# microsoft/demikernel

Hardware: AMD Instinct MI355X
Metric: GB/s packet bytes checksummed+parsed (device-resident) (higher is better)
Workload: dtype u8; 1 GPU; 1M x 1500B IPv4/TCP, 1024 flows, device-resident; frames_per_gpu=1048576, global_frames=1048576, parallelism=packet-shard x1, collective=none

## Files before the change

### demikernel_amd/csrc/tcp_kernels.hip

```cpp
#include <hip/hip_runtime.h>
#include <rocprim/device/device_radix_sort.hpp>
#include <rocprim/iterator/counting_iterator.hpp>
#include <rocprim/warp/warp_scan.hpp>

#include <algorithm>
#include <climits>
#include <cerrno>
#include <cstdlib>
#include <cstddef>
#include <cstring>

#include "../../include/dk_diag.h"
#include "../../include/dk_tcp.h"
#include "tcp_order.h"

namespace dk_tcp {
namespace {

constexpr uint32_t kBlock = 256;
constexpr uint32_t kBatch = 8;

using SortConfig = rocprim::radix_sort_config<rocprim::default_config, rocprim::default_config,
                                              rocprim::default_config, 0>;

__device__ __forceinline__ bool lt(uint32_t a, uint32_t b) { return (int32_t)(a - b) < 0; }
__device__ __forceinline__ bool le(uint32_t a, uint32_t b) { return (int32_t)(a - b) <= 0; }
__device__ __forceinline__ bool ge(uint32_t a, uint32_t b) { return (int32_t)(a - b) >= 0; }

struct Params {
    const uint32_t* meta;
    const uint32_t* flow_id;
    const uint32_t* seq;
    const uint32_t* ack;
    const uint32_t* payload;
    uint32_t n;
    dk_tcp_conn* conns;
    uint32_t nconns;
    uint32_t* keys;
    uint32_t* skeys;
    uint32_t* svals;
    uint4* rec;
    uint32_t* range;
    uint32_t* cls;
    uint32_t* open_until;
    uint4* scan_sum;
    int* scan_ends;
    uint32_t* scan_idx;
    uint4* scan_rec;
    uint4* scan_post;
    uint32_t* scan_head;
    uint32_t* shape;
    uint32_t* shape_host;
    uint32_t call;
    dk_tcp_out out;
};
constexpr uint32_t kNoConn = 0xFFFFFFFFu;

__global__ __launch_bounds__(kBlock) void dk_tcp_key_kernel(Params P) {
    const uint32_t i = blockIdx.x * kBlock + threadIdx.x;
    if (i >= P.n) return;
    const uint32_t meta = P.meta[i], pay = P.payload[i], seq = P.seq[i];
    uint32_t key = 2 * P.nconns, cls = kNoConn;
    uint8_t act = DK_TCP_SKIP;
    if ((meta & 0xFFu) == DK_V_OK_TCP) {
        const uint32_t f = P.flow_id[i];
        if (f < P.nconns) {
            static_assert(offsetof(dk_tcp_conn, state) == 0 && offsetof(dk_tcp_conn, receive_next) == 4 &&
                              offsetof(dk_tcp_conn, reader_next) == 8 && offsetof(dk_tcp_conn, buffer_size) == 12,
                          "dk_tcp_conn layout");
            const uint4 h = *reinterpret_cast<const uint4*>(P.conns + f);
            const uint32_t state = h.x;
            if (state != DK_TCP_NONE) key = 2 * f;
            const uint32_t bufsz = h.w, rn0 = h.y, wend = h.z + bufsz;
            if (state == DK_TCP_ESTABLISHED && wend - rn0 <= bufsz && bufsz < 0x40000000u) {
                const uint32_t flags = (meta >> 16) & 0xFFu, len = pay >> 16;
                const uint32_t full = len + ((flags >> 1) & 1u) + (flags & 1u);
                const uint32_t seg_end = full ? seq + (full - 1) : seq;
                const uint32_t lim = 0x7FFFFFFFu - bufsz - 0x20000u;
                if (seq - wend - 1u < lim) act = DK_TCP_OUT_OF_WINDOW;
                else if (rn0 - seg_end - 1u < lim) act = DK_TCP_DUPLICATE;
                if (act != DK_TCP_SKIP) {
                    cls = f;
                    key = 2 * f + 1;
                }
            }
        }
    }
    P.keys[i] = key;
    P.cls[i] = cls;
    P.rec[i] = make_uint4(seq, P.ack[i], meta, pay);
    if (key == 2 * P.nconns || cls != kNoConn) {
        P.out.action[i] = act;
        P.out.view[i] = dk_tcp_view{i, pay & 0xFFFFu, pay >> 16};
    }
}

constexpr uint32_t kShapeBlocks = 64;
__global__ __launch_bounds__(kBlock) void dk_tcp_fix_kernel(Params P) {
    __shared__ uint32_t s_cnt[kBlock / 64];
    const uint32_t i = blockIdx.x * kBlock + threadIdx.x;
    bool stored = false;
    if (i < P.n) {
        const uint32_t c = P.cls[i];
        if (c != kNoConn && i >= P.open_until[c]) P.out.action[i] = DK_TCP_UNPROCESSED;
        else stored = blockIdx.x < kShapeBlocks && c == kNoConn && P.out.action[i] == DK_TCP_STORED;
    }
    if (blockIdx.x >= kShapeBlocks) return;
    const uint64_t m = __ballot(stored);
    if ((threadIdx.x & 63u) == 0) s_cnt[threadIdx.x / 64] = (uint32_t)__popcll(m);
    __syncthreads();
    if (threadIdx.x == 0) {
        uint32_t sum = 0;
        for (uint32_t w = 0; w < kBlock / 64; w++) sum += s_cnt[w];
        const uint32_t nb = min(gridDim.x, kShapeBlocks);
        const unsigned long long old = atomicAdd(reinterpret_cast<unsigned long long*>(P.shape),
                                                 (1ull << 40) | (unsigned long long)sum);
        if ((uint32_t)(old >> 40) == nb - 1) {
            const uint32_t total = (uint32_t)(old & ((1ull << 40) - 1)) + sum;
            atomicExch(reinterpret_cast<unsigned long long*>(P.shape), 0ull);
            __hip_atomic_store(P.shape_host + 0, total, __ATOMIC_RELAXED, __HIP_MEMORY_SCOPE_SYSTEM);
            __hip_atomic_store(P.shape_host + 1, min(P.n, nb * kBlock), __ATOMIC_RELAXED, __HIP_MEMORY_SCOPE_SYSTEM);
            __hip_atomic_store(P.shape_host + 2, P.call, __ATOMIC_RELAXED, __HIP_MEMORY_SCOPE_SYSTEM);
        }
    }
}

__global__ __launch_bounds__(kBlock) void dk_tcp_range_kernel(Params P) {
    const uint32_t c = blockIdx.x * kBlock + threadIdx.x;
    if (c > 2 * P.nconns) return;
    uint32_t lo = 0, hi = P.n;
    while (lo < hi) {
        const uint32_t mid = lo + (hi - lo) / 2;
        if (P.skeys[mid] < c)
            lo = mid + 1;
        else
            hi = mid;
    }
    P.range[c] = lo;
}

constexpr uint32_t kSortBlock = 512, kSortWaves = kSortBlock / 64, kSortTile = 8192, kSortSub = kSortTile / kSortWaves;
#ifndef DK_TCP_SORT_ROWS
#define DK_TCP_SORT_ROWS 255
#endif
constexpr uint32_t kSortMaxRows = DK_TCP_SORT_ROWS, kSortMaxBuckets = 2 * kSortMaxRows + 1;
struct SortPass {
    const uint32_t* kin;
    const uint32_t* vin;
    uint32_t* kout;
    uint32_t* vout;
    uint32_t* H;
    uint32_t shift, mask, nbuck;
};

__device__ __forceinline__ uint64_t digit_group(uint32_t d, bool live, uint32_t nbits) {
    uint64_t same = __ballot(live);
    for (uint32_t bit = 0; bit < nbits; bit++) {
        const uint64_t ones = __ballot(live && ((d >> bit) & 1u));
        same &= ((d >> bit) & 1u) ? ones : ~ones;
    }
    return same;
}
constexpr uint32_t kSortRounds = kSortSub / 64;
constexpr uint32_t kSortGroupBits = 4;

__device__ __forceinline__ void sort_load_keys(const SortPass& S, uint32_t s0, uint32_t s1, uint32_t lane,
                                               uint32_t (&kr)[kSortRounds]) {
#pragma unroll
    for (uint32_t r = 0; r < kSortRounds; r++) {
        const uint32_t i = s0 + r * 64 + lane;
        kr[r] = i < s1 ? S.kin[i] : 0u;
    }
}
__device__ __forceinline__ void sort_count_keys(const SortPass& S, uint32_t s0, uint32_t s1, uint32_t lane,
                                                const uint32_t (&kr)[kSortRounds], uint32_t* cnt, uint32_t nbits) {
    const uint64_t lt = (1ull << lane) - 1;
#pragma unroll
    for (uint32_t r = 0; r < kSortRounds; r++) {
        const bool live = s0 + r * 64 + lane < s1;
        const uint32_t d = (kr[r] >> S.shift) & S.mask;
        if (nbits <= kSortGroupBits) {
            const uint64_t same = digit_group(d, live, nbits);
            if (live && !(same & lt)) atomicAdd(&cnt[d], (uint32_t)__popcll(same));
        } else if (live) {
            atomicAdd(&cnt[d], 1u);
        }
    }
}

__global__ __launch_bounds__(kSortBlock) void dk_tcp_sort_count_kernel(uint32_t n, SortPass S) {
    __shared__ uint32_t hist[kSortMaxBuckets];
    const uint32_t b = blockIdx.x, nb = gridDim.x, tid = threadIdx.x, lane = tid & 63, wv = tid >> 6;
    const uint32_t nbits = 32u - (uint32_t)__builtin_clz(S.mask | 1u);
    uint32_t kr[kSortRounds];
    const uint32_t s0 = b * kSortTile + wv * kSortSub, s1 = min(n, s0 + kSortSub);
    sort_load_keys(S, s0, s1, lane, kr);
    for (uint32_t k = tid; k < S.nbuck; k += kSortBlock) hist[k] = 0;
    __syncthreads();
    sort_count_keys(S, s0, s1, lane, kr, hist, nbits);
    __syncthreads();
    for (uint32_t k = tid; k < S.nbuck; k += kSortBlock) S.H[(size_t)k * nb + b] = hist[k];
}

constexpr uint32_t kSortScanBlock = 1024, kSortScanPer = 12, kSortScanRow = kSortScanPer + 1;
__global__ __launch_bounds__(kSortScanBlock) void dk_tcp_sort_scan_kernel(uint32_t* H, uint32_t m, uint32_t nb,
                                                                          uint32_t* range) {
// ... 276 lines not shown
    if (data.len > 0 || fin) {
        if (seg_start != w.rn) {
            action = DK_TCP_STORED;
            if (seg_len > 0) {
                if (fin) {
                    seg_len -= 1;
                    w.fin_pending = 1;
                    w.fin_seq = seg_end;
                    seg_end -= 1;
                    fin = false;
                }
                if (seg_len > 0) action = ooo_store(s, w, seg_start, seg_end, data);
            }
        } else {
            action = DK_TCP_DELIVERED;
            if (receive_data(s, w, data, o)) fin = true;
        }
    }
    if (fin) {
        o.push(dk_tcp_view{DK_TCP_REF_EOF, 0, 0}, w);
        w.rn += 1;
        w.state = DK_TCP_CLOSED;
        return DK_TCP_FIN;
    }
    return action;
}

__global__ __launch_bounds__(kWalkBlock) void dk_tcp_walk_kernel(Params P) {
    __shared__ uint32_t lds[4 * DK_TCP_OOO_MAX * kWalkBlock];
    const uint32_t c = blockIdx.x * kWalkBlock + threadIdx.x;
    if (c >= P.nconns) return;
    dk_tcp_conn* t = P.conns + c;
    const uint32_t k0 = P.range[2 * c], cnt = P.range[2 * c + 1] - k0, all = P.range[2 * c + 2] - k0;
    const uint32_t d0 = k0 + DK_TCP_DELIV_EXTRA * c;
    P.out.deliv_start[c] = d0;
    Walk w{t->state, t->receive_next, t->reader_next, t->buffer_size, t->send_next, t->fin_pending, t->fin_seq,
           min(t->ooo_count, DK_TCP_OOO_MAX)};
    Store s{lds + threadIdx.x};
    for (uint32_t k = 0; k < w.nooo; k++) s.set(k, t->ooo_start[k], t->ooo[k]);
    uint32_t open_until = w.state == DK_TCP_ESTABLISHED ? 0xFFFFFFFFu : 0u;
    Out o{P.out.deliv + d0, 0, all + DK_TCP_DELIV_EXTRA};
    uint32_t ia[kBatch], ib[kBatch], ic[kBatch];
    uint4 gb[kBatch], gc[kBatch];
#pragma unroll
    for (uint32_t j = 0; j < kBatch; j++) {
        ib[j] = j < cnt ? P.svals[k0 + j] : 0u;
        ia[j] = kBatch + j < cnt ? P.svals[k0 + kBatch + j] : 0u;
    }
#pragma unroll
    for (uint32_t j = 0; j < kBatch; j++)
        if (j < cnt) gb[j] = P.rec[ib[j]];
    for (uint32_t k = 0; k < cnt; k += kBatch) {
#pragma unroll
        for (uint32_t j = 0; j < kBatch; j++) {
            gc[j] = gb[j];
            ic[j] = ib[j];
        }
        if (k + kBatch < cnt) {
#pragma unroll
            for (uint32_t j = 0; j < kBatch; j++) {
                if (k + kBatch + j < cnt) gb[j] = P.rec[ia[j]];
                ib[j] = ia[j];
            }
        }
        if (k + 2 * kBatch < cnt) {
#pragma unroll
            for (uint32_t j = 0; j < kBatch; j++)
                if (k + 2 * kBatch + j < cnt) ia[j] = P.svals[k0 + k + 2 * kBatch + j];
        }
#pragma unroll
        for (uint32_t j = 0; j < kBatch; j++) {
            if (k + j >= cnt) break;
            if (w.state != DK_TCP_ESTABLISHED) {
                P.out.action[ic[j]] = DK_TCP_UNPROCESSED;
                P.out.view[ic[j]] = dk_tcp_view{ic[j], gc[j].w & 0xFFFFu, gc[j].w >> 16};
                continue;
            }
            dk_tcp_view v;
            P.out.action[ic[j]] = (uint8_t)process(s, w, gc[j], ic[j], o, v);
            P.out.view[ic[j]] = v;
            if (w.state != DK_TCP_ESTABLISHED) open_until = ic[j] + 1;
        }
    }
    P.open_until[c] = open_until;
    t->state = w.state;
    t->receive_next = w.rn;
    t->fin_pending = w.fin_pending;
    t->fin_seq = w.fin_seq;
    t->ooo_count = w.nooo;
    for (uint32_t k = 0; k < DK_TCP_OOO_MAX; k++) {
        const bool live = k < w.nooo;
        t->ooo_start[k] = live ? s.start(k) : 0u;
        t->ooo[k] = live ? s.view(k) : dk_tcp_view{0, 0, 0};
    }
    P.out.deliv_count[c] = o.n;
}

constexpr uint32_t kWave = 64;

using WaveScan = rocprim::warp_scan<uint32_t, kWave>;

constexpr uint32_t kRingH = 6, kIdxSlots = 16, kRecSlots = 8;
static_assert(2 * kRingH + 1 <= kIdxSlots && kRingH + 1 <= kRecSlots, "ring slots cover the windows in flight");
static_assert(2 * kRingH - 2 == 10, "the s_waitcnt immediate below");
typedef __attribute__((address_space(3))) void lds_void;
typedef unsigned u32x4 __attribute__((ext_vector_type(4)));
template <class T>
__device__ __forceinline__ uint32_t lds_addr(T* p) {
    return (uint32_t)(uintptr_t)(__attribute__((address_space(3))) T*)p;
}
__device__ __forceinline__ uint32_t lds_read_u32(uint32_t a) {
    uint32_t v;
    asm volatile("ds_read_b32 %0, %1\n\ts_waitcnt lgkmcnt(0)" : "=v"(v) : "v"(a) : "memory");
    return v;
}
__device__ __forceinline__ void lds_read_window(uint32_t a_i, uint32_t a_g, uint32_t a_f, uint32_t& i, uint4& g,
                                                uint32_t& f) {
    u32x4 q;
    asm volatile("ds_read_b32 %0, %3\n\tds_read_b128 %1, %4\n\tds_read_b32 %2, %5\n\ts_waitcnt lgkmcnt(0)"
                 : "=&v"(i), "=&v"(q), "=&v"(f)
                 : "v"(a_i), "v"(a_g), "v"(a_f)
                 : "memory");
    g = make_uint4(q.x, q.y, q.z, q.w);
}

struct Seg {
    uint32_t x, off, len, dend, seg_end;
    bool have, simple, syn, ack_ok;
    uint8_t fast_action;
    __device__ __forceinline__ Seg(uint4 g, bool have_, uint32_t snd) {
        const uint32_t flags = (g.z >> 16) & 0xFFu;
        x = g.x;
        off = g.w & 0xFFFFu;
        len = g.w >> 16;
        have = have_;
        simple = have && !(flags & 0x07u);
        syn = have && (flags & 0x07u) == 0x02u;
        ack_ok = (flags & 0x10u) && le(g.y, snd);
        fast_action = !(flags & 0x10u) ? DK_TCP_NO_ACK : !ack_ok ? DK_TCP_ACK_UNSENT : len > 0 ? DK_TCP_DELIVERED : DK_TCP_NO_DATA;
        dend = x + len;
        const uint32_t full = len + ((flags >> 1) & 1u) + (flags & 1u);
        seg_end = full ? x + (full - 1) : x;
    }
    __device__ __forceinline__ bool cand(bool beyond, uint32_t wend) const {
        return simple && !beyond && ack_ok && len > 0 && !ge(dend - 1u, wend);
    }
};
struct Verdict {
    bool ok;
    uint8_t act;
    uint32_t voff, vlen;
};
__device__ __forceinline__ Verdict classify(const Seg& q, uint32_t rn, uint32_t wend, bool beyond, uint32_t nooo,
                                            uint32_t front, uint32_t fin_pending, uint32_t fin_seq,
                                            bool syn_reach = false) {
    const bool drains = q.ack_ok && q.len > 0 && ((nooo && q.dend == front) || (fin_pending && q.dend == fin_seq));
    const bool at = q.x == rn, before = lt(q.x, rn), dup = before && lt(q.seg_end, rn);
    const bool oow = !at && !before && ge(q.x, wend);
    const bool past = !at && !before && !oow;
    const bool data_in = !ge(q.dend - 1u, wend), plain = q.simple && !beyond && !drains;
    const bool syn_ok = q.syn && (at || past) && !ge(q.seg_end, wend);
    const uint32_t send1 = q.seg_end + 1u;
    const bool syn_part_ok = syn_reach && q.syn && before && !dup && !ge(q.seg_end, wend) &&
                             !(q.ack_ok && ((nooo && send1 == front) || (fin_pending && send1 == fin_seq)));
    const bool ok = dup || oow || syn_ok || syn_part_ok || (at && plain && (q.len == 0 || data_in)) ||
                    (before && plain && data_in) || (past && beyond) ||
                    (past && q.simple && q.fast_action != DK_TCP_DELIVERED);
// ... 66 lines not shown
            const uint32_t a_f = process(s, w, gf, i_f, o, v);
            if (lane == 0) {
                P.out.action[i_f] = (uint8_t)a_f;
                P.out.view[i_f] = v;
            }
            if (w.state != DK_TCP_ESTABLISHED) open_until = i_f + 1;
            lo = f + 1;
        }
    }
};

__device__ __forceinline__ void ring_walk(const Params& P, WaveWalk& W, uint32_t (&sidx)[kIdxSlots][kWave],
                                          uint4 (&srec)[kRecSlots][kWave], uint32_t k0, uint32_t cnt, uint32_t v0,
                                          uint32_t v1) {
    const uint32_t lane = W.lane, last = cnt ? cnt - 1 : 0u;
    const auto idx_dma = [&](uint32_t u) {
        __builtin_amdgcn_global_load_lds((const void*)(P.svals + k0 + min(u * kWave + lane, last)),
                                         (lds_void*)&sidx[u % kIdxSlots][0], 4, 0, 0);
    };
    const auto rec_dma = [&](uint32_t u, uint32_t fi) {
        __builtin_amdgcn_global_load_lds((const void*)(P.rec + fi), (lds_void*)&srec[u % kRecSlots][0], 16, 0, 0);
    };
    const auto idx_at = [&](uint32_t u) { return lds_addr(&sidx[u % kIdxSlots][lane]); };
    if (v0 >= v1) return;
    for (uint32_t u = v0; u < v0 + kRingH; u++) idx_dma(u);
    asm volatile("s_waitcnt vmcnt(0)" ::: "memory");
    for (uint32_t u = v0; u < v0 + kRingH; u++) {
        rec_dma(u, lds_read_u32(idx_at(u)));
        idx_dma(u + kRingH);
    }
    for (uint32_t v = v0; v < v1; v++) {
        asm volatile("s_waitcnt vmcnt(10)" ::: "memory");
        uint32_t i, fi;
        uint4 g;
        lds_read_window(idx_at(v), lds_addr(&srec[v % kRecSlots][lane]), idx_at(v + kRingH), i, g, fi);
        rec_dma(v + kRingH, fi);
        idx_dma(v + 2 * kRingH);
        W.window(v * kWave, i, g);
    }
    asm volatile("s_waitcnt vmcnt(0)" ::: "memory");
}

#define DK_U(x) (uint32_t) __builtin_amdgcn_readfirstlane((int)(x))

template <bool kRing>
__global__ __launch_bounds__(kWave) void dk_tcp_wave_walk_kernel(Params P) {
    __shared__ WaveScan::storage_type scan_tmp;
    __shared__ uint32_t sidx[kRing ? kIdxSlots : 1][kWave];
    __shared__ uint4 srec[kRing ? kRecSlots : 1][kWave];
    const uint32_t c = blockIdx.x, lane = threadIdx.x;
    dk_tcp_conn* t = P.conns + c;
    const uint32_t k0 = P.range[2 * c], cnt = P.range[2 * c + 1] - k0, all = P.range[2 * c + 2] - k0;
    const uint32_t d0 = k0 + DK_TCP_DELIV_EXTRA * c;
    const Walk w0{DK_U(t->state), DK_U(t->receive_next), DK_U(t->reader_next), DK_U(t->buffer_size),
                  DK_U(t->send_next), DK_U(t->fin_pending), DK_U(t->fin_seq), DK_U(min(t->ooo_count, DK_TCP_OOO_MAX))};
    RegStore s0{0u, 0u, 0u, 0u, lane};
    if (lane < w0.nooo) {
        const dk_tcp_view v = t->ooo[lane];
        s0 = RegStore{t->ooo_start[lane], v.ref, v.off, v.len, lane};
    }
    WaveWalk W{P, w0, s0, Out{P.out.deliv + d0, 0, all + DK_TCP_DELIV_EXTRA},
               w0.state == DK_TCP_ESTABLISHED ? 0xFFFFFFFFu : 0u, w0.reader + w0.bufsz, cnt, lane, scan_tmp};
    const uint32_t last = cnt ? cnt - 1 : 0u;
    if constexpr (kRing) {
        ring_walk(P, W, sidx, srec, k0, cnt, 0u, (uint32_t)(((uint64_t)cnt + kWave - 1) / kWave));
    } else {
        const auto idx = [&](uint32_t u) { return P.svals[k0 + min(u * kWave + lane, last)]; };
        uint32_t i = 0, i1 = 0;
        uint4 g = make_uint4(0u, 0u, 0u, 0u);
        if (cnt) {
            i = idx(0);
            i1 = idx(1);
            g = P.rec[i];
        }
        for (uint32_t v = 0; v * kWave < cnt; v++) {
            const uint32_t i2 = idx(v + 2);
            const uint4 g1 = P.rec[i1];
            W.window(v * kWave, i, g);
            i = i1;
            i1 = i2;
            g = g1;
        }
    }
    if (lane == 0) {
        P.out.deliv_start[c] = d0;
        P.open_until[c] = W.open_until;
        t->state = W.w.state;
        t->receive_next = W.w.rn;
        t->fin_pending = W.w.fin_pending;
        t->fin_seq = W.w.fin_seq;
        t->ooo_count = W.w.nooo;
        P.out.deliv_count[c] = W.o.n;
    }
    if (lane < DK_TCP_OOO_MAX) {
        const bool live = lane < W.w.nooo;
        t->ooo_start[lane] = live ? W.s.st : 0u;
        t->ooo[lane] = live ? dk_tcp_view{W.s.rf, W.s.of, W.s.ln} : dk_tcp_view{0, 0, 0};
    }
}

struct alignas(16) Baton {
    uint32_t turn;
    uint32_t epoch;
    uint32_t rn, n;
    uint32_t state, nooo, front;
    uint32_t fin_pending, fin_seq, open_until;
};
__device__ __forceinline__ uint32_t lds_relaxed(uint32_t* p) {
    return __hip_atomic_load(p, __ATOMIC_RELAXED, __HIP_MEMORY_SCOPE_WORKGROUP);
}
__device__ __forceinline__ void baton_poll(const Baton* bt, uint32_t& turn, uint32_t& epoch, uint32_t& rn,
                                           uint32_t& n) {
    const uint32_t a = (uint32_t)reinterpret_cast<uintptr_t>(bt);
    uint32_t t, e;
    uint2 rv;
    asm volatile(
        "ds_read_b32 %0, %3\n\t"
        "ds_read_b32 %1, %3 offset:4\n\t"
        "ds_read_b64 %2, %3 offset:8\n\t"
        "s_waitcnt lgkmcnt(0)"
        : "=v"(t), "=v"(e), "=v"(rv)
        : "v"(a)
        : "memory");
    turn = DK_U(t);
    epoch = DK_U(e);
    rn = DK_U(rv.x);
    n = DK_U(rv.y);
}
__device__ __forceinline__ void baton_pass(Baton* bt, uint32_t turn, uint32_t rn, uint32_t n) {
    const uint32_t a = (uint32_t)reinterpret_cast<uintptr_t>(bt);
    const uint2 rv = make_uint2(rn, n);
    asm volatile(
        "ds_write_b64 %0, %1 offset:8\n\t"
        "ds_write_b32 %0, %2"
        :
        : "v"(a), "v"(rv), "v"(turn)
        : "memory");
}

template <uint32_t kRelayWaves>
__global__ __launch_bounds__(kRelayWaves * kWave) void dk_tcp_relay_walk_kernel(Params P) {
    __shared__ WaveScan::storage_type scan_tmp[kRelayWaves];
    __shared__ Baton bt;
    __shared__ uint32_t sto[4][DK_TCP_OOO_MAX];
    const uint32_t c = blockIdx.x, lane = threadIdx.x & (kWave - 1), wv = DK_U(threadIdx.x / kWave);
    dk_tcp_conn* t = P.conns + c;
    const uint32_t k0 = P.range[2 * c], cnt = P.range[2 * c + 1] - k0, all = P.range[2 * c + 2] - k0;
    const uint32_t d0 = k0 + DK_TCP_DELIV_EXTRA * c, cap = all + DK_TCP_DELIV_EXTRA;
    dk_tcp_view* const dv = P.out.deliv + d0;
    const uint32_t rn0 = DK_U(t->receive_next), reader = DK_U(t->reader_next), bufsz = DK_U(t->buffer_size),
                   snd = DK_U(t->send_next), wend = reader + bufsz;
    if (wv == 0) {
        const uint32_t state = t->state, nooo = min(t->ooo_count, DK_TCP_OOO_MAX);
        if (lane < DK_TCP_OOO_MAX) {
            const dk_tcp_view e = t->ooo[lane];
            sto[0][lane] = t->ooo_start[lane];
            sto[1][lane] = e.ref;
            sto[2][lane] = e.off;
            sto[3][lane] = e.len;
        }
        if (lane == 0)
            bt = Baton{0u, 0u, rn0, 0u, state, nooo, nooo ? t->ooo_start[0] : 0u, t->fin_pending, t->fin_seq,
                       state == DK_TCP_ESTABLISHED ? 0xFFFFFFFFu : 0u};
    }
    __syncthreads();
    const uint32_t nwin = (uint32_t)(((uint64_t)cnt + kWave - 1) / kWave), last = cnt ? cnt - 1 : 0u;
    const auto idx = [&](uint32_t v) { return P.svals[k0 + min(v * kWave + lane, last)]; };
    uint32_t i = 0, i1 = 0;
    uint4 g = make_uint4(0u, 0u, 0u, 0u);
// ... 75 lines not shown
                    const dk_tcp_view view{i, r.voff, r.vlen};
                    P.out.action[i] = r.act;
                    P.out.view[i] = view;
                    if (r.act == DK_TCP_DELIVERED && n_now + before < cap) dv[n_now + before] = view;
                }
                i = i1;
                i1 = i2;
                g = g1;
                continue;
            }
        }
        const Baton b{v, 0u, DK_U(bt.rn), DK_U(bt.n), DK_U(bt.state), DK_U(bt.nooo), DK_U(bt.front),
                      DK_U(bt.fin_pending), DK_U(bt.fin_seq), DK_U(bt.open_until)};
        const bool plain_state = b.state == DK_TCP_ESTABLISHED && b.nooo < DK_TCP_OOO_MAX;
        const uint32_t R = b.rn - rn0;
        uint32_t f = 0;
        Verdict r{};
        uint64_t pmk = 0;
        if (plain_state) {
            r = classify(q, rn0 + max(R, pm), wend, false, b.nooo, b.front, b.fin_pending, b.fin_seq, syn_r);
            const uint64_t bad = __ballot(q.have && !r.ok);
            f = bad ? (uint32_t)__builtin_ctzll(bad) : kWave;
            pmk = __ballot(q.have && lane < f && r.act == DK_TCP_DELIVERED);
            if (!bad && lane == 0) baton_pass(&bt, v + 1, rn0 + max(R, wmax), b.n + (uint32_t)__builtin_popcountll(pmk));
        }
        const uint32_t i2 = idx(v + 2 * kRelayWaves);
        const uint4 g1 = P.rec[i1];
        if (q.have && lane < f) {
            const uint32_t before =
                __builtin_amdgcn_mbcnt_hi((uint32_t)(pmk >> 32), __builtin_amdgcn_mbcnt_lo((uint32_t)pmk, 0u));
            const dk_tcp_view view{i, r.voff, r.vlen};
            P.out.action[i] = r.act;
            P.out.view[i] = view;
            if (r.act == DK_TCP_DELIVERED && b.n + before < cap) dv[b.n + before] = view;
        }
        if (f < kWave) {
            RegStore s{0u, 0u, 0u, 0u, lane};
            if (lane < b.nooo) s = RegStore{sto[0][lane], sto[1][lane], sto[2][lane], sto[3][lane], lane};
            const uint32_t rn_f = rn0 + max(R, (uint32_t)__builtin_amdgcn_readlane(pm, f));
            WaveWalk W{P, Walk{b.state, rn_f, reader, bufsz, snd, b.fin_pending, b.fin_seq, b.nooo}, s,
                       Out{dv, b.n + (uint32_t)__builtin_popcountll(pmk), cap}, b.open_until, wend, cnt, lane,
                       scan_tmp[wv]};
            if (plain_state) {
                const uint4 gf = make_uint4(__builtin_amdgcn_readlane(g.x, f), __builtin_amdgcn_readlane(g.y, f),
                                            __builtin_amdgcn_readlane(g.z, f), __builtin_amdgcn_readlane(g.w, f));
                const uint32_t i_f = __builtin_amdgcn_readlane(i, f);
                dk_tcp_view vf;
                const uint32_t a_f = process(W.s, W.w, gf, i_f, W.o, vf);
                if (lane == 0) {
                    P.out.action[i_f] = (uint8_t)a_f;
                    P.out.view[i_f] = vf;
                }
                if (W.w.state != DK_TCP_ESTABLISHED) W.open_until = i_f + 1;
                W.window(base, i, g, f + 1);
            } else {
                W.window(base, i, g, 0);
            }
            if (lane < DK_TCP_OOO_MAX) {
                sto[0][lane] = W.s.st;
                sto[1][lane] = W.s.rf;
                sto[2][lane] = W.s.of;
                sto[3][lane] = W.s.ln;
            }
            const uint32_t front = W.w.nooo ? W.s.start(0) : 0u;
            if (lane == 0) {
                bt.state = W.w.state;
                bt.rn = W.w.rn;
                bt.nooo = W.w.nooo;
                bt.front = front;
                bt.fin_pending = W.w.fin_pending;
                bt.fin_seq = W.w.fin_seq;
                bt.n = W.o.n;
                bt.open_until = W.open_until;
                bt.epoch = bt.epoch + 1;
            }
            if (lane == 0) __hip_atomic_store(&bt.turn, v + 1, __ATOMIC_RELEASE, __HIP_MEMORY_SCOPE_WORKGROUP);
        }
        i = i1;
        i1 = i2;
        g = g1;
    }
    __syncthreads();
    if (wv == 0) {
        if (lane == 0) {
            P.out.deliv_start[c] = d0;
            P.open_until[c] = bt.open_until;
            t->state = bt.state;
            t->receive_next = bt.rn;
            t->fin_pending = bt.fin_pending;
            t->fin_seq = bt.fin_seq;
            t->ooo_count = bt.nooo;
            P.out.deliv_count[c] = bt.n;
        }
        if (lane < DK_TCP_OOO_MAX) {
            const bool live = lane < bt.nooo;
            t->ooo_start[lane] = live ? sto[0][lane] : 0u;
            t->ooo[lane] = live ? dk_tcp_view{sto[1][lane], sto[2][lane], sto[3][lane]} : dk_tcp_view{0, 0, 0};
        }
    }
}

struct Pre {
    uint32_t pm, key, wmax;
    bool cand, syn_r, synd;
};
__device__ __forceinline__ Pre pre_window(const Seg& q, uint32_t rn0, uint32_t wend, WaveScan::storage_type& scan) {
    Pre r;
    r.cand = q.cand(false, wend);
    const uint32_t key1 = r.cand && lt(rn0, q.dend) ? q.dend - rn0 : 0u;
    uint32_t pm1;
    WaveScan().exclusive_scan(key1, pm1, 0u, scan, rocprim::maximum<uint32_t>());
    r.syn_r = q.syn && !ge(q.seg_end, wend) && (int)(q.x - rn0) < (int)pm1;
    r.synd = r.syn_r && q.ack_ok;
    r.key = r.synd && lt(rn0, q.seg_end + 1u) ? max(key1, q.seg_end + 1u - rn0) : key1;
    WaveScan().exclusive_scan(r.key, r.pm, 0u, scan, rocprim::maximum<uint32_t>());
    r.wmax = (uint32_t)__builtin_amdgcn_readlane(max(r.pm, r.key), kWave - 1);
    return r;
}
struct ConnHead {
    uint32_t state, rn0, reader, bufsz, snd, wend, nooo, front, finp, fins;
    __device__ __forceinline__ explicit ConnHead(const dk_tcp_conn* t) {
        state = DK_U(t->state);
        rn0 = DK_U(t->receive_next);
        reader = DK_U(t->reader_next);
        bufsz = DK_U(t->buffer_size);
        snd = DK_U(t->send_next);
        wend = reader + bufsz;
        nooo = DK_U(min(t->ooo_count, DK_TCP_OOO_MAX));
        front = nooo ? DK_U(t->ooo_start[0]) : 0u;
        finp = DK_U(t->fin_pending);
        fins = DK_U(t->fin_seq);
    }
};
__device__ __forceinline__ uint32_t scan_ws(const Params& P, uint32_t c) { return P.range[2 * c] / kWave + c; }

#ifndef DK_TCP_SCAN_STATS
#define DK_TCP_SCAN_STATS 0
#endif
constexpr uint32_t kScanBlock = 256, kScanWaves = kScanBlock / kWave;
#ifndef DK_TCP_SCAN_DEPTH
#define DK_TCP_SCAN_DEPTH 8
#endif
constexpr uint32_t kScanDepth = DK_TCP_SCAN_DEPTH;
#ifndef DK_TCP_SCAN_PREFETCH
#define DK_TCP_SCAN_PREFETCH 1
#endif
constexpr bool kScanPrefetch = DK_TCP_SCAN_PREFETCH != 0;
constexpr uint32_t kScanSum = 3;
constexpr uint32_t kScanLow = 4;
constexpr uint32_t kScanPost = 1024;
constexpr uint32_t kScanRingRun = 8, kScanRingRunMax = 512;
__global__ __launch_bounds__(kScanBlock) void dk_tcp_scan_pre_kernel(Params P) {
    __shared__ WaveScan::storage_type scan_tmp[kScanWaves];
    const uint32_t c = blockIdx.y, lane = threadIdx.x & (kWave - 1), wv = DK_U(threadIdx.x / kWave);
    const dk_tcp_conn* t = P.conns + c;
    const uint32_t k0 = P.range[2 * c], cnt = P.range[2 * c + 1] - k0;
    const uint32_t nwin = (uint32_t)(((uint64_t)cnt + kWave - 1) / kWave), last = cnt ? cnt - 1 : 0u;
    if (blockIdx.x * kScanWaves >= nwin) return;
    const ConnHead h(t);
    const uint32_t ws0 = scan_ws(P, c);
    for (uint32_t v = blockIdx.x * kScanWaves + wv; v < nwin; v += gridDim.x * kScanWaves) {
        const uint32_t base = v * kWave, lim = min(cnt - base, kWave);
        const uint32_t i = P.svals[k0 + min(base + lane, last)];
        const uint4 g = P.rec[i];
        P.scan_idx[(size_t)(ws0 + v) * kWave + lane] = i;
        P.scan_rec[(size_t)(ws0 + v) * kWave + lane] = g;
        const Seg q(g, lane < lim, h.snd);
        const Pre pr = pre_window(q, h.rn0, h.wend, scan_tmp[wv]);
        const int xr = (int)(q.x - h.rn0), er = (int)(q.seg_end - h.rn0), dr = (int)(q.dend - h.rn0), pmi = (int)pr.pm;
// ... 185 lines not shown
            }
            if (W.w.state != DK_TCP_ESTABLISHED) W.open_until = i_f + 1;
            W.window(base, i, g, fl + 1);
            w = W.w;
            s = W.s;
            n = W.o.n;
            open_until = W.open_until;
        }
        v++;
#if DK_TCP_SCAN_STATS
        ck_slow += wall_clock64() - ck_s;
#endif
    };
    const auto ring_run = [&](uint32_t v1) {
#if DK_TCP_SCAN_STATS
        st_ring += v1 - v;
        st_runs++;
        const uint64_t ck_r = wall_clock64();
#endif
        for (uint32_t u = v + lane; u < v1; u += kWave) P.scan_post[ws0 + u] = make_uint4(0u, 0u, 0u, 0u);
        WaveWalk W{P, w, s, Out{dv, n, cap}, open_until, h.wend, cnt, lane, scan_tmp[0]};
        ring_walk(P, W, sidx, srec, k0, cnt, v, v1);
        w = W.w;
        s = W.s;
        n = W.o.n;
        open_until = W.open_until;
        v = v1;
#if DK_TCP_SCAN_STATS
        ck_ring += wall_clock64() - ck_r;
#endif
    };
    Batch b[kScanDepth];
    uint32_t last_slow = 0xFFFFFFFEu, run = kScanRingRun;
    uint32_t pre = 0xFFFFFFFFu;
    while (v < nwin && !stale) {
#if DK_TCP_SCAN_STATS
        st_restart++;
#endif
        bool more = true;
        while (more && v < nwin) {
            if (v + kScanDepth * kWave > vflush + kScanPost) flush_post();
            if (pre != v) {
#pragma unroll
                for (uint32_t j = 0; j < kScanDepth; j++)
                    if (v + j * kWave < nwin) load_batch(v + j * kWave, b[j]);
            }
            pre = 0xFFFFFFFFu;
#pragma unroll
            for (uint32_t j = 0; j < kScanDepth; j++)
                if (more && batch_step(b[j]) < kWave) more = false;
        }
        flush_post();
        if (v >= nwin) break;
        if (v == last_slow + 1) {
            ring_run(v + min(run, nwin - v));
            last_slow = v - 1;
            run = min(2 * run, kScanRingRunMax);
        } else {
            if (v - last_slow > kWave) run = kScanRingRun;
            last_slow = v;
            if (kScanPrefetch) {
#pragma unroll
                for (uint32_t j = 0; j < kScanDepth; j++)
                    if (v + 1 + j * kWave < nwin) load_batch(v + 1 + j * kWave, b[j]);
                pre = v + 1;
            }
            slow_window();
        }
        vflush = v;
        const uint32_t front = w.nooo ? s.start(0) : 0u;
        stale = w.state != h.state || w.nooo != h.nooo || front != h.front || w.fin_pending != h.finp ||
                w.fin_seq != h.fins;
    }
    if (v < nwin) ring_run(nwin);
#if DK_TCP_SCAN_STATS
    if (lane == 0)
        printf("{\"scan_stats\": 1, \"conn\": %u, \"windows\": %u, \"batch_steps\": %u, \"full_steps\": %u, "
               "\"slow_windows\": %u, \"ring_windows\": %u, \"ring_runs\": %u, \"restarts\": %u, \"stale\": %u, "
               "\"us_total\": %.2f, \"us_batch_steps\": %.2f, \"us_slow\": %.2f, \"us_ring\": %.2f}\n",
               c, nwin, st_batch, st_full, st_slow, st_ring, st_runs, st_restart, (uint32_t)stale,
               (double)(wall_clock64() - ck_t0) / 100.0, (double)ck_batch / 100.0, (double)ck_slow / 100.0,
               (double)ck_ring / 100.0);
#endif
    if (lane == 0) {
        P.out.deliv_start[c] = d0;
        P.open_until[c] = open_until;
        t->state = w.state;
        t->receive_next = w.rn;
        t->fin_pending = w.fin_pending;
        t->fin_seq = w.fin_seq;
        t->ooo_count = w.nooo;
        P.out.deliv_count[c] = n;
    }
    if (lane < DK_TCP_OOO_MAX) {
        const bool live = lane < w.nooo;
        t->ooo_start[lane] = live ? s.st : 0u;
        t->ooo[lane] = live ? dk_tcp_view{s.rf, s.of, s.ln} : dk_tcp_view{0, 0, 0};
    }
}

__global__ __launch_bounds__(kScanBlock) void dk_tcp_scan_post_kernel(Params P) {
    __shared__ WaveScan::storage_type scan_tmp[kScanWaves];
    const uint32_t c = blockIdx.y, lane = threadIdx.x & (kWave - 1), wv = DK_U(threadIdx.x / kWave);
    const uint32_t k0 = P.range[2 * c], cnt = P.range[2 * c + 1] - k0, all = P.range[2 * c + 2] - k0;
    const uint32_t nwin = (uint32_t)(((uint64_t)cnt + kWave - 1) / kWave), last = cnt ? cnt - 1 : 0u;
    if (blockIdx.x * kScanWaves >= nwin) return;
    const uint32_t d0 = k0 + DK_TCP_DELIV_EXTRA * c, cap = all + DK_TCP_DELIV_EXTRA;
    dk_tcp_view* const dv = P.out.deliv + d0;
    const uint32_t ws0 = scan_ws(P, c);
    const uint32_t* hd = P.scan_head + 8 * c;
    const uint32_t rn0 = DK_U(hd[0]), wend = DK_U(hd[1]), snd = DK_U(hd[2]), nooo = DK_U(hd[3]), front = DK_U(hd[4]),
                   finp = DK_U(hd[5]), fins = DK_U(hd[6]);
    for (uint32_t v = blockIdx.x * kScanWaves + wv; v < nwin; v += gridDim.x * kScanWaves) {
        const uint4 po = P.scan_post[ws0 + v];
        const uint32_t i = P.scan_idx[(size_t)(ws0 + v) * kWave + lane];
        const uint4 g = P.scan_rec[(size_t)(ws0 + v) * kWave + lane];
        if (DK_U(po.z) != 1u) continue;
        const uint32_t base = v * kWave, lim = min(cnt - base, kWave);
        const Seg q(g, lane < lim, snd);
        const Pre pr = pre_window(q, rn0, wend, scan_tmp[wv]);
        const int Rq = (int)DK_U(po.x), pmi = (int)pr.pm;
        const int er = (int)(q.seg_end - rn0), dr = (int)(q.dend - rn0);
        const int E = pr.synd ? er + 1 : dr;
        const bool deliv0 = (pr.cand || pr.synd) && pmi < E;
        const uint64_t pk = __ballot(deliv0 && Rq < E);
        const uint32_t n0 = DK_U(po.y);
        const Verdict r = classify(q, rn0 + (uint32_t)max(Rq, pmi), wend, false, nooo, front, finp, fins, pr.syn_r);
        const uint32_t before =
            __builtin_amdgcn_mbcnt_hi((uint32_t)(pk >> 32), __builtin_amdgcn_mbcnt_lo((uint32_t)pk, 0u));
        if (q.have) {
            const dk_tcp_view view{i, r.voff, r.vlen};
            P.out.action[i] = r.act;
            P.out.view[i] = view;
            if (r.act == DK_TCP_DELIVERED && n0 + before < cap) dv[n0 + before] = view;
        }
    }
}
#undef DK_U

constexpr uint32_t kWaveWalkMinSegs = 8;
constexpr uint32_t kScanMinSegs = 16 * kWave;
#ifndef DK_TCP_SCAN_MAX_CONNS
#define DK_TCP_SCAN_MAX_CONNS 256
#endif
#ifndef DK_TCP_DEEP_MAX_CONNS
#define DK_TCP_DEEP_MAX_CONNS 2048
#endif
constexpr uint32_t kDeepAheadMaxConns = DK_TCP_DEEP_MAX_CONNS;
constexpr uint32_t kShapeMinConns = 16, kShapeStoredDen = 1024;
enum Walker { kLaneWalk = 0, kWaveWalk = 1, kRelayWalk = 2, kScanWalk = 3 };
Walker pick_walk(uint32_t n, uint32_t nconns, int force, bool reordered) {
    if (nconns > (1u << 24)) return kLaneWalk;
    if (force == 3 && nconns > 65535) return kRelayWalk;
    if (force >= 0 && force <= 3) return (Walker)force;
    if ((uint64_t)n < (uint64_t)kWaveWalkMinSegs * nconns) return kLaneWalk;
    if ((uint64_t)n >= (uint64_t)kScanMinSegs * nconns && nconns <= DK_TCP_SCAN_MAX_CONNS &&
        !(reordered && nconns >= kShapeMinConns))
        return kScanWalk;
    return kWaveWalk;
}

struct DeviceGuard {
    int prev = -1;
    explicit DeviceGuard(int dev) {
        if (hipGetDevice(&prev) != hipSuccess) prev = -1;
        if (prev != dev) (void)hipSetDevice(dev);
    }
    ~DeviceGuard() {
        if (prev >= 0) (void)hipSetDevice(prev);
    }
};

template <class T>
int grow(T*& p, size_t& cap, size_t n) {
    if (cap >= n) return 0;
    if (p) (void)hipFree(p);
    p = nullptr;
    cap = 0;
    if (hipMalloc(reinterpret_cast<void**>(&p), std::max<size_t>(n, 1) * sizeof(T)) != hipSuccess) return ENOMEM;
    cap = n;
    return 0;
}

}
}

struct dk_tcp_ctx {
    int device = 0;
    int walk = -1;
    int relay_waves = 8;
    hipEvent_t last = nullptr;
    hipStream_t last_stream = nullptr;
    bool used = false;
    uint32_t *keys = nullptr, *skeys = nullptr, *svals = nullptr, *range = nullptr, *cls = nullptr, *open_until = nullptr;
    size_t keys_cap = 0, skeys_cap = 0, svals_cap = 0, range_cap = 0, cls_cap = 0, open_cap = 0;
    uint32_t* csort = nullptr;
    size_t csort_cap = 0;
    uint4* rec = nullptr;
    size_t rec_cap = 0;
    uint8_t* temp = nullptr;
    size_t temp_cap = 0;
    uint4 *scan_sum = nullptr, *scan_post = nullptr;
    int* scan_ends = nullptr;
    uint32_t* scan_idx = nullptr;
    uint4* scan_rec = nullptr;
    size_t scan_idx_cap = 0, scan_rec_cap = 0;
    uint32_t* scan_head = nullptr;
    size_t scan_sum_cap = 0, scan_post_cap = 0, scan_ends_cap = 0, scan_head_cap = 0;
    uint32_t* shape = nullptr;
    volatile uint32_t* shape_host = nullptr;
    uint32_t* shape_host_dev = nullptr;
    uint32_t calls = 0;
    uint32_t seen = 0;
    bool reordered = false;
    int last_walk = -1;
    int sort = -1;
    int last_sort = -1;
    bool ord_live = false;
    uint32_t ord_n = 0, ord_nconns = 0, ord_call = 0;
    dk_tcp_ack_state ack;
    dk_tcp_emit_state emit;
    dk_tcp_cc_state cc;
};

int dk_tcp_ctx_order(dk_tcp_ctx* t, dk_tcp_order* o) {
    if (!t || !o) return EINVAL;
    *o = dk_tcp_order{t->device, t->svals, t->range, t->rec, t->ord_live, t->ord_n, t->ord_nconns, t->ord_call,
                      t->last, &t->last_stream, &t->used, &t->ack, &t->emit, &t->cc};
    return 0;
}

extern "C" {

int dk_tcp_ctx_create(int32_t device, dk_tcp_ctx** out) {
    if (!out) return EINVAL;
    *out = nullptr;
    int nd = 0;
    if (hipGetDeviceCount(&nd) != hipSuccess || device < 0 || device >= nd) return EINVAL;
    dk_tcp::DeviceGuard g(device);
    dk_tcp_ctx* t = new dk_tcp_ctx();
    t->device = device;
    void* hs = nullptr;
    if (hipEventCreateWithFlags(&t->last, hipEventDisableTiming) != hipSuccess) {
        delete t;
        return EINVAL;
    }
    if (hipMalloc(&t->shape, 2 * sizeof(uint32_t)) != hipSuccess || hipMemset(t->shape, 0, 8) != hipSuccess ||
        hipHostMalloc(&hs, 4 * sizeof(uint32_t), hipHostMallocMapped | hipHostMallocCoherent) != hipSuccess ||
        hipHostGetDevicePointer(reinterpret_cast<void**>(&t->shape_host_dev), hs, 0) != hipSuccess) {
        if (hs) (void)hipHostFree(hs);
        if (t->shape) (void)hipFree(t->shape);
        (void)hipEventDestroy(t->last);
        delete t;
        return ENOMEM;
    }
    t->shape_host = static_cast<volatile uint32_t*>(hs);
    t->shape_host[0] = t->shape_host[1] = t->shape_host[2] = 0;
    *out = t;
    return 0;
}

int dk_diag_tcp_last_walk(const dk_tcp_ctx* t) { return t ? t->last_walk : -1; }

int dk_diag_tcp_last_sort(const dk_tcp_ctx* t) { return t ? t->last_sort : -1; }

int dk_diag_tcp_set_walk(dk_tcp_ctx* t, int32_t walk, int32_t relay_waves) {
    if (!t || walk < -1 || walk > 3) return EINVAL;
    t->walk = walk;
    t->relay_waves = relay_waves == 4 || relay_waves == 16 ? relay_waves : 8;
    return 0;
}

int dk_diag_tcp_set_sort(dk_tcp_ctx* t, int32_t sort) {
    if (!t || (sort != -1 && sort != 1)) return EINVAL;
    t->sort = sort;
    return 0;
}

void dk_tcp_ctx_destroy(dk_tcp_ctx* t) {
    if (!t) return;
    dk_tcp::DeviceGuard g(t->device);
    if (t->used) (void)hipEventSynchronize(t->last);
    for (void* p : {(void*)t->keys, (void*)t->skeys, (void*)t->svals, (void*)t->range, (void*)t->rec, (void*)t->temp,
                    (void*)t->cls, (void*)t->open_until, (void*)t->scan_sum, (void*)t->scan_post, (void*)t->scan_ends,
                    (void*)t->scan_idx, (void*)t->scan_rec,
                    (void*)t->scan_head, (void*)t->shape, (void*)t->csort, t->ack.scratch, t->emit.scratch})
        if (p) (void)hipFree(p);
    if (t->shape_host) (void)hipHostFree(const_cast<uint32_t*>(t->shape_host));
    (void)hipEventDestroy(t->last);
    delete t;
}

int dk_tcp_rx_process(dk_tcp_ctx* t, const dk_rx_results* rx, uint32_t n, dk_tcp_conn* conns, uint32_t nconns,
                      const dk_tcp_out* out, void* stream) {
    using namespace dk_tcp;
    if (!t || !rx || !out) return EINVAL;
    if (n && (!rx->meta || !rx->flow_id || !rx->payload || !rx->tcp_seq || !rx->tcp_ack || !out->action || !out->view))
        return EINVAL;
    if (nconns && (!conns || !out->deliv || !out->deliv_start || !out->deliv_count)) return EINVAL;
    if (reinterpret_cast<uintptr_t>(conns) & 15) return EINVAL;
    if (n > 0x7FFFFFFFu || nconns > 0x7FFFFFFFu ||
        (uint64_t)n + (uint64_t)DK_TCP_DELIV_EXTRA * nconns > 0xFFFFFFFFull)
        return EINVAL;
    t->ord_live = false;
    if (n == 0 && nconns == 0) {
        t->last_sort = -1;
        t->ord_live = true, t->ord_n = 0, t->ord_nconns = 0, t->ord_call++;
        return 0;
    }
    DeviceGuard g(t->device);
    const hipStream_t s = (hipStream_t)stream;
    int rc = 0;
    if (t->used && t->last_stream != s && hipStreamWaitEvent(s, t->last, 0) != hipSuccess) return EINVAL;
    const bool grows = t->keys_cap < n || t->rec_cap < n || t->range_cap < 2 * (size_t)nconns + 1 || t->cls_cap < n ||
                       t->open_cap < nconns;
    if (t->used && grows && hipEventSynchronize(t->last) != hipSuccess) return EINVAL;
    if ((rc = grow(t->keys, t->keys_cap, n)) || (rc = grow(t->skeys, t->skeys_cap, n)) ||
        (rc = grow(t->svals, t->svals_cap, n)) || (rc = grow(t->rec, t->rec_cap, n)) ||
        (rc = grow(t->range, t->range_cap, 2 * (size_t)nconns + 1)) || (rc = grow(t->cls, t->cls_cap, n)) ||
        (rc = grow(t->open_until, t->open_cap, nconns)))
        return rc;
    if (t->calls != t->seen && t->shape_host[2] != t->seen) {
        const uint32_t call = t->shape_host[2];
        const uint32_t stored = t->shape_host[0], segs = t->shape_host[1];
        if (call == t->shape_host[2] && call != t->seen) {
            t->seen = call;
            t->reordered = (uint64_t)stored * dk_tcp::kShapeStoredDen >= (uint64_t)std::max(segs, 1u);
        }
    }
    const dk_tcp::Walker walker = nconns ? dk_tcp::pick_walk(n, nconns, t->walk, t->reordered) : dk_tcp::kLaneWalk;
    t->last_walk = (int)walker;
    if (walker == dk_tcp::kScanWalk) {
        const size_t nw = (size_t)n / 64 + nconns + 1;
        if (t->used &&
            (t->scan_sum_cap < dk_tcp::kScanSum * nw || t->scan_ends_cap < nw * 64 || t->scan_head_cap < 8ull * nconns ||
             t->scan_idx_cap < nw * 64 || t->scan_rec_cap < nw * 64) &&
            hipEventSynchronize(t->last) != hipSuccess)
            return EINVAL;
        if ((rc = grow(t->scan_sum, t->scan_sum_cap, dk_tcp::kScanSum * nw)) || (rc = grow(t->scan_post, t->scan_post_cap, nw)) ||
            (rc = grow(t->scan_ends, t->scan_ends_cap, nw * 64)) || (rc = grow(t->scan_idx, t->scan_idx_cap, nw * 64)) ||
            (rc = grow(t->scan_rec, t->scan_rec_cap, nw * 64)) ||
            (rc = grow(t->scan_head, t->scan_head_cap, 8 * (size_t)nconns)))
            return rc;
    }
    int bits = 1;
    while (bits < 32 && (1ull << bits) <= 2ull * nconns) bits++;
    const rocprim::counting_iterator<uint32_t> index(0);
    const uint32_t nkeys = 2 * nconns + 1, ntiles = (n + dk_tcp::kSortTile - 1) / dk_tcp::kSortTile;
    const bool csort = nconns && n && nconns <= dk_tcp::kSortMaxRows && t->sort != 1;
    t->last_sort = nconns && n ? (csort ? 0 : 1) : -1;
    if (csort) {
        const size_t hb = (size_t)nkeys * ntiles;
        if (t->used && t->csort_cap < hb && hipEventSynchronize(t->last) != hipSuccess) return EINVAL;
        if ((rc = grow(t->csort, t->csort_cap, hb))) return rc;
    } else {
        size_t sort_bytes = 0;
        if (rocprim::radix_sort_pairs<SortConfig>(nullptr, sort_bytes, t->keys, t->skeys, index, t->svals, n, 0, bits,
                                                  s) != hipSuccess)
            return EINVAL;
        if (t->used && t->temp_cap < sort_bytes && hipEventSynchronize(t->last) != hipSuccess) return EINVAL;
        if ((rc = grow(t->temp, t->temp_cap, sort_bytes))) return rc;
    }

    Params P{};
    P.meta = rx->meta;
    P.flow_id = rx->flow_id;
    P.seq = rx->tcp_seq;
    P.ack = rx->tcp_ack;
    P.payload = rx->payload;
    P.n = n;
    P.conns = conns;
    P.nconns = nconns;
    P.keys = t->keys;
    P.skeys = t->skeys;
    P.svals = t->svals;
    P.rec = t->rec;
    P.range = t->range;
    P.cls = t->cls;
    P.open_until = t->open_until;
    P.scan_sum = t->scan_sum;
    P.scan_post = t->scan_post;
    P.scan_ends = t->scan_ends;
    P.scan_idx = t->scan_idx;
    P.scan_rec = t->scan_rec;
    P.scan_head = t->scan_head;
    P.shape = t->shape;
    P.shape_host = t->shape_host_dev;
    P.call = t->calls + 1;
    P.out = *out;
    const dim3 gn((n + kBlock - 1) / kBlock), gr((2 * nconns + kBlock) / kBlock), gc((nconns + kWalkBlock - 1) / kWalkBlock);
    if (n) hipLaunchKernelGGL(dk_tcp_key_kernel, gn, dim3(kBlock), 0, s, P);
    if (csort) {
        const auto pass = [&](const SortPass& S, uint32_t* range) {
            hipLaunchKernelGGL(dk_tcp_sort_count_kernel, dim3(ntiles), dim3(kSortBlock), 0, s, n, S);
            hipLaunchKernelGGL(dk_tcp_sort_scan_kernel, dim3(1), dim3(kSortScanBlock), 0, s, S.H, S.nbuck * ntiles,
                               ntiles, range);
            hipLaunchKernelGGL(dk_tcp_sort_scatter_kernel, dim3(ntiles), dim3(kSortBlock), 0, s, n, S);
        };
        uint32_t mask = 1;
        while (mask < nkeys - 1) mask = 2 * mask + 1;
        pass(SortPass{t->keys, nullptr, nullptr, t->svals, t->csort, 0u, mask, nkeys}, t->range);
    } else {
        if (n) {
            size_t b = t->temp_cap;
            if (rocprim::radix_sort_pairs<SortConfig>(t->temp, b, t->keys, t->skeys, index, t->svals, n, 0, bits, s) !=
                hipSuccess)
                return EINVAL;
        }
        if (nconns) hipLaunchKernelGGL(dk_tcp_range_kernel, gr, dim3(kBlock), 0, s, P);
    }
    if (nconns) {
        switch (walker) {
            case kScanWalk: {
                const uint32_t per = (uint32_t)(((uint64_t)n / kWave / nconns + kScanWaves) / kScanWaves);
                const dim3 gs(std::min<uint32_t>(std::max<uint32_t>(per, 1u), 65535u), nconns);
                hipLaunchKernelGGL(dk_tcp_scan_pre_kernel, gs, dim3(kScanBlock), 0, s, P);
                hipLaunchKernelGGL(dk_tcp_scan_kernel, dim3(nconns), dim3(kWave), 0, s, P);
                hipLaunchKernelGGL(dk_tcp_scan_post_kernel, gs, dim3(kScanBlock), 0, s, P);
                break;
            }
            case kRelayWalk:
                if (t->relay_waves == 4)
                    hipLaunchKernelGGL(dk_tcp_relay_walk_kernel<4>, dim3(nconns), dim3(4 * kWave), 0, s, P);
                else if (t->relay_waves == 16)
                    hipLaunchKernelGGL(dk_tcp_relay_walk_kernel<16>, dim3(nconns), dim3(16 * kWave), 0, s, P);
                else
                    hipLaunchKernelGGL(dk_tcp_relay_walk_kernel<8>, dim3(nconns), dim3(8 * kWave), 0, s, P);
                break;
            case kWaveWalk:
                if (nconns <= kDeepAheadMaxConns)
                    hipLaunchKernelGGL(dk_tcp_wave_walk_kernel<true>, dim3(nconns), dim3(kWave), 0, s, P);
                else
                    hipLaunchKernelGGL(dk_tcp_wave_walk_kernel<false>, dim3(nconns), dim3(kWave), 0, s, P);
                break;
            default:
                hipLaunchKernelGGL(dk_tcp_walk_kernel, gc, dim3(kWalkBlock), 0, s, P);
        }
    }
    if (n && nconns) {
        hipLaunchKernelGGL(dk_tcp_fix_kernel, gn, dim3(kBlock), 0, s, P);
        t->calls++;
    }
    if (hipGetLastError() != hipSuccess) return EINVAL;
    if (hipEventRecord(t->last, s) != hipSuccess) return EINVAL;
    t->last_stream = s;
    t->used = true;
    t->ord_live = true, t->ord_n = n, t->ord_nconns = nconns, t->ord_call++;
    return 0;
}

}
```

Before: 6646 GB/s.

## Fold unprocessed fixup into walkers and replace range binary search with boundary scatter

Drops the per-packet cls and open_until arrays. Each walker now marks the classified tail of its flow (sorted entries past cnt) as unprocessed when the connection closes, and the full-grid fix kernel shrinks to a shape-count kernel of at most 64 blocks. The binary-search range kernel is replaced, when keys fit, by a kernel that writes range boundaries by reading adjacent sorted keys. This removes one full pass over n packets plus two per-packet writes, at the cost of walkers looping over classified entries themselves.

```diff
diff --git a/demikernel_amd/csrc/tcp_kernels.hip b/demikernel_amd/csrc/tcp_kernels.hip
--- a/demikernel_amd/csrc/tcp_kernels.hip
+++ b/demikernel_amd/csrc/tcp_kernels.hip
@@ -41,8 +41,6 @@
     uint32_t* svals;
     uint4* rec;
     uint32_t* range;
-    uint32_t* cls;
-    uint32_t* open_until;
     uint4* scan_sum;
     int* scan_ends;
     uint32_t* scan_idx;
@@ -54,13 +52,12 @@
     uint32_t call;
     dk_tcp_out out;
 };
-constexpr uint32_t kNoConn = 0xFFFFFFFFu;
 
 __global__ __launch_bounds__(kBlock) void dk_tcp_key_kernel(Params P) {
     const uint32_t i = blockIdx.x * kBlock + threadIdx.x;
     if (i >= P.n) return;
     const uint32_t meta = P.meta[i], pay = P.payload[i], seq = P.seq[i];
-    uint32_t key = 2 * P.nconns, cls = kNoConn;
+    uint32_t key = 2 * P.nconns;
     uint8_t act = DK_TCP_SKIP;
     if ((meta & 0xFFu) == DK_V_OK_TCP) {
         const uint32_t f = P.flow_id[i];
@@ -79,33 +76,32 @@
                 const uint32_t lim = 0x7FFFFFFFu - bufsz - 0x20000u;
                 if (seq - wend - 1u < lim) act = DK_TCP_OUT_OF_WINDOW;
                 else if (rn0 - seg_end - 1u < lim) act = DK_TCP_DUPLICATE;
-                if (act != DK_TCP_SKIP) {
-                    cls = f;
-                    key = 2 * f + 1;
-                }
+                if (act != DK_TCP_SKIP) key = 2 * f + 1;
             }
         }
     }
     P.keys[i] = key;
-    P.cls[i] = cls;
     P.rec[i] = make_uint4(seq, P.ack[i], meta, pay);
-    if (key == 2 * P.nconns || cls != kNoConn) {
+    if (key == 2 * P.nconns || (key & 1u)) {
         P.out.action[i] = act;
         P.out.view[i] = dk_tcp_view{i, pay & 0xFFFFu, pay >> 16};
     }
 }
 
+__device__ __forceinline__ void close_classified(const Params& P, uint32_t k1, uint32_t k2, uint32_t open_until,
+                                                 uint32_t lane, uint32_t step) {
+    if (open_until == 0xFFFFFFFFu) return;
+    for (uint32_t k = k1 + lane; k < k2; k += step) {
+        const uint32_t i = P.svals[k];
+        if (i >= open_until) P.out.action[i] = DK_TCP_UNPROCESSED;
+    }
+}
+
 constexpr uint32_t kShapeBlocks = 64;
-__global__ __launch_bounds__(kBlock) void dk_tcp_fix_kernel(Params P) {
+__global__ __launch_bounds__(kBlock) void dk_tcp_shape_kernel(Params P) {
     __shared__ uint32_t s_cnt[kBlock / 64];
     const uint32_t i = blockIdx.x * kBlock + threadIdx.x;
-    bool stored = false;
-    if (i < P.n) {
-        const uint32_t c = P.cls[i];
-        if (c != kNoConn && i >= P.open_until[c]) P.out.action[i] = DK_TCP_UNPROCESSED;
-        else stored = blockIdx.x < kShapeBlocks && c == kNoConn && P.out.action[i] == DK_TCP_STORED;
-    }
-    if (blockIdx.x >= kShapeBlocks) return;
+    const bool stored = i < P.n && P.out.action[i] == DK_TCP_STORED;
     const uint64_t m = __ballot(stored);
     if ((threadIdx.x & 63u) == 0) s_cnt[threadIdx.x / 64] = (uint32_t)__popcll(m);
     __syncthreads();
@@ -122,6 +118,27 @@
             __hip_atomic_store(P.shape_host + 1, min(P.n, nb * kBlock), __ATOMIC_RELAXED, __HIP_MEMORY_SCOPE_SYSTEM);
             __hip_atomic_store(P.shape_host + 2, P.call, __ATOMIC_RELAXED, __HIP_MEMORY_SCOPE_SYSTEM);
         }
+    }
+}
+
+constexpr uint32_t kBoundsLaneGap = 4;
+__global__ __launch_bounds__(kBlock) void dk_tcp_bounds_kernel(Params P) {
+    const uint32_t p = blockIdx.x * kBlock + threadIdx.x, lane = threadIdx.x & 63u;
+    const bool live = p <= P.n;
+    uint32_t k = 0, end = 0;
+    if (live) {
+        k = p ? P.skeys[p - 1] + 1 : 0u;
+        end = (p < P.n ? P.skeys[p] : 2 * P.nconns) + 1;
+    }
+    const bool wide = end - k > kBoundsLaneGap;
+    if (!wide)
+        for (; k < end; k++) P.range[k] = p;
+    for (uint64_t m = __ballot(wide); m; m &= m - 1) {
+        const uint32_t l = (uint32_t)__builtin_ctzll(m);
+        const uint32_t k0 = (uint32_t)__builtin_amdgcn_readlane((int)k, l);
+        const uint32_t k1 = (uint32_t)__builtin_amdgcn_readlane((int)end, l);
+        const uint32_t pl = (uint32_t)__builtin_amdgcn_readlane((int)p, l);
+        for (uint32_t j = k0 + lane; j < k1; j += 64) P.range[j] = pl;
     }
 }
 
@@ -564,7 +581,7 @@
             if (w.state != DK_TCP_ESTABLISHED) open_until = ic[j] + 1;
         }
     }
-    P.open_until[c] = open_until;
+    close_classified(P, k0 + cnt, k0 + all, open_until, 0u, 1u);
     t->state = w.state;
     t->receive_next = w.rn;
     t->fin_pending = w.fin_pending;
@@ -797,9 +814,9 @@
             g = g1;
         }
     }
+    close_classified(P, k0 + cnt, k0 + all, W.open_until, lane, kWave);
     if (lane == 0) {
         P.out.deliv_start[c] = d0;
-        P.open_until[c] = W.open_until;
         t->state = W.w.state;
         t->receive_next = W.w.rn;
         t->fin_pending = W.w.fin_pending;
@@ -1041,9 +1058,9 @@
     }
     __syncthreads();
     if (wv == 0) {
+        close_classified(P, k0 + cnt, k0 + all, bt.open_until, lane, kWave);
         if (lane == 0) {
             P.out.deliv_start[c] = d0;
-            P.open_until[c] = bt.open_until;
             t->state = bt.state;
             t->receive_next = bt.rn;
             t->fin_pending = bt.fin_pending;
@@ -1395,9 +1412,9 @@
                (double)(wall_clock64() - ck_t0) / 100.0, (double)ck_batch / 100.0, (double)ck_slow / 100.0,
                (double)ck_ring / 100.0);
 #endif
+    close_classified(P, k0 + cnt, k0 + all, open_until, lane, kWave);
     if (lane == 0) {
         P.out.deliv_start[c] = d0;
-        P.open_until[c] = open_until;
         t->state = w.state;
         t->receive_next = w.rn;
         t->fin_pending = w.fin_pending;
@@ -1505,8 +1522,8 @@
     hipEvent_t last = nullptr;
     hipStream_t last_stream = nullptr;
     bool used = false;
-    uint32_t *keys = nullptr, *skeys = nullptr, *svals = nullptr, *range = nullptr, *cls = nullptr, *open_until = nullptr;
-    size_t keys_cap = 0, skeys_cap = 0, svals_cap = 0, range_cap = 0, cls_cap = 0, open_cap = 0;
+    uint32_t *keys = nullptr, *skeys = nullptr, *svals = nullptr, *range = nullptr;
+    size_t keys_cap = 0, skeys_cap = 0, svals_cap = 0, range_cap = 0;
     uint32_t* csort = nullptr;
     size_t csort_cap = 0;
     uint4* rec = nullptr;
@@ -1595,9 +1612,9 @@
     dk_tcp::DeviceGuard g(t->device);
     if (t->used) (void)hipEventSynchronize(t->last);
     for (void* p : {(void*)t->keys, (void*)t->skeys, (void*)t->svals, (void*)t->range, (void*)t->rec, (void*)t->temp,
-                    (void*)t->cls, (void*)t->open_until, (void*)t->scan_sum, (void*)t->scan_post, (void*)t->scan_ends,
-                    (void*)t->scan_idx, (void*)t->scan_rec,
-                    (void*)t->scan_head, (void*)t->shape, (void*)t->csort, t->ack.scratch, t->emit.scratch})
+                    (void*)t->scan_sum, (void*)t->scan_post, (void*)t->scan_ends, (void*)t->scan_idx,
+                    (void*)t->scan_rec, (void*)t->scan_head, (void*)t->shape, (void*)t->csort, t->ack.scratch,
+                    t->emit.scratch})
         if (p) (void)hipFree(p);
     if (t->shape_host) (void)hipHostFree(const_cast<uint32_t*>(t->shape_host));
     (void)hipEventDestroy(t->last);
@@ -1625,13 +1642,11 @@
     const hipStream_t s = (hipStream_t)stream;
     int rc = 0;
     if (t->used && t->last_stream != s && hipStreamWaitEvent(s, t->last, 0) != hipSuccess) return EINVAL;
-    const bool grows = t->keys_cap < n || t->rec_cap < n || t->range_cap < 2 * (size_t)nconns + 1 || t->cls_cap < n ||
-                       t->open_cap < nconns;
+    const bool grows = t->keys_cap < n || t->rec_cap < n || t->range_cap < 2 * (size_t)nconns + 1;
     if (t->used && grows && hipEventSynchronize(t->last) != hipSuccess) return EINVAL;
     if ((rc = grow(t->keys, t->keys_cap, n)) || (rc = grow(t->skeys, t->skeys_cap, n)) ||
         (rc = grow(t->svals, t->svals_cap, n)) || (rc = grow(t->rec, t->rec_cap, n)) ||
-        (rc = grow(t->range, t->range_cap, 2 * (size_t)nconns + 1)) || (rc = grow(t->cls, t->cls_cap, n)) ||
-        (rc = grow(t->open_until, t->open_cap, nconns)))
+        (rc = grow(t->range, t->range_cap, 2 * (size_t)nconns + 1)))
         return rc;
     if (t->calls != t->seen && t->shape_host[2] != t->seen) {
         const uint32_t call = t->shape_host[2];
@@ -1689,8 +1704,6 @@
     P.svals = t->svals;
     P.rec = t->rec;
     P.range = t->range;
-    P.cls = t->cls;
-    P.open_until = t->open_until;
     P.scan_sum = t->scan_sum;
     P.scan_post = t->scan_post;
     P.scan_ends = t->scan_ends;
@@ -1720,7 +1733,10 @@
                 hipSuccess)
                 return EINVAL;
         }
-        if (nconns) hipLaunchKernelGGL(dk_tcp_range_kernel, gr, dim3(kBlock), 0, s, P);
+        if (nconns && nkeys <= n)
+            hipLaunchKernelGGL(dk_tcp_bounds_kernel, dim3(n / kBlock + 1), dim3(kBlock), 0, s, P);
+        else if (nconns)
+            hipLaunchKernelGGL(dk_tcp_range_kernel, gr, dim3(kBlock), 0, s, P);
     }
     if (nconns) {
         switch (walker) {
@@ -1751,7 +1767,7 @@
         }
     }
     if (n && nconns) {
-        hipLaunchKernelGGL(dk_tcp_fix_kernel, gn, dim3(kBlock), 0, s, P);
+        hipLaunchKernelGGL(dk_tcp_shape_kernel, dim3(std::min(gn.x, kShapeBlocks)), dim3(kBlock), 0, s, P);
         t->calls++;
     }
     if (hipGetLastError() != hipSuccess) return EINVAL;
```

Result: no change. 6637 GB/s (-0.1%).
